# sonbui25/Multimodal-Aspect-Category-Sentiment-Analysis

Hardware: AMD Instinct MI355X
Metric: train samples/sec (fwd+bwd+step) FCMF seq128x36ROI (higher is better)
Workload: dtype bf16; 1 GPU; FCMF-base fine-tune step, BASELINE configs[1]: batch 64 reviews x 6 aspects per GPU, seq 128, 7 images x (49 patches + 36 ROIs), precomputed ResNet-152 features, dropout 0.1, clip 1.0 + 4-group AdamW + linear schedule; global_batch=64, per_gpu_batch=64, seq_len=128, parallelism=dp1, sample_unit=1 review = 6 aspect forwards

## Files before the change

multimodal-aspect-category-sentiment-analysis_amd/csrc/attn_mfma.hip:

```cpp
#include "common.h"
#include <cstdlib>

constexpr int AD = 64;
constexpr int AT = 128;
constexpr int TILE_B = AT * AD * 2;

__device__ __forceinline__ int vkey(int r) { return ((r >> 1) & 1) | (((r >> 3) & 1) << 1); }
__device__ __forceinline__ int off64(int r, int c8) { return r * 128 + ((((c8 >> 1) ^ vkey(r))) << 5) + ((c8 & 1) << 4); }
__device__ __forceinline__ int key16(int r) { return ((r & 7) << 1) ^ (((r >> 3) & 1) * 9); }
__device__ __forceinline__ int off128(int r, int ch) { return r * 256 + ((ch ^ key16(r)) << 4); }
__device__ __forceinline__ int offp(int r, int ch) { return r * 256 + ((ch ^ (r & 15)) << 4); }

__device__ __forceinline__ int off64p(int r, int c8) { return r * 128 + ((((c8 >> 1) ^ ((r >> 1) & 3))) << 5) + ((c8 & 1) << 4); }

typedef bf16x4 __attribute__((address_space(3))) * lds_v4_t;

__device__ __forceinline__ void stage_tile(char* lds, const bf16_t* __restrict__ src, int64_t ld, int rows, int tid) {
#pragma unroll
  for (int i = 0; i < 4; ++i) {
    const int c = tid + 256 * i, r = c >> 3, c8 = c & 7;
    uint4 v = make_uint4(0, 0, 0, 0);
    if (r < rows) v = *reinterpret_cast<const uint4*>(src + (int64_t)r * ld + c8 * 8);
    *reinterpret_cast<uint4*>(lds + off64(r, c8)) = v;
  }
}
__device__ __forceinline__ void stage_tile_p(char* lds, const bf16_t* __restrict__ src, int64_t ld, int rows, int tid) {
#pragma unroll
  for (int i = 0; i < 4; ++i) {
    const int c = tid + 256 * i, r = c >> 3, c8 = c & 7;
    uint4 v = make_uint4(0, 0, 0, 0);
    if (r < rows) v = *reinterpret_cast<const uint4*>(src + (int64_t)r * ld + c8 * 8);
    *reinterpret_cast<uint4*>(lds + off64p(r, c8)) = v;
  }
}
__device__ __forceinline__ bf16x8 frag_tr64p(const char* lds, int c0, int s, int lane) {
  const int g4 = lane >> 4, i16 = lane & 15, q4 = i16 >> 2, p = i16 & 3;
  const int r = 32 * s + 4 * g4 + q4, c8 = (c0 >> 3) + (p >> 1);
  bf16x4 lo = __builtin_amdgcn_ds_read_tr16_b64_v4bf16((lds_v4_t)(lds + off64p(r, c8) + (p & 1) * 8));
  bf16x4 hi = __builtin_amdgcn_ds_read_tr16_b64_v4bf16((lds_v4_t)(lds + off64p(r + 16, c8) + (p & 1) * 8));
  bf16x8 o;
  o[0] = lo[0]; o[1] = lo[1]; o[2] = lo[2]; o[3] = lo[3]; o[4] = hi[0]; o[5] = hi[1]; o[6] = hi[2]; o[7] = hi[3];
  return o;
}
struct TileRegs { uint4 v[4]; };
__device__ __forceinline__ TileRegs load_tile(const bf16_t* __restrict__ src, int64_t ld, int rows, int tid) {
  TileRegs t;
#pragma unroll
  for (int i = 0; i < 4; ++i) {
    const int c = tid + 256 * i, r = c >> 3, c8 = c & 7;
    t.v[i] = make_uint4(0, 0, 0, 0);
    if (r < rows) t.v[i] = *reinterpret_cast<const uint4*>(src + (int64_t)r * ld + c8 * 8);
  }
  return t;
}
template <bool PERMUTED>
__device__ __forceinline__ void store_tile(char* lds, const TileRegs& t, int tid) {
#pragma unroll
  for (int i = 0; i < 4; ++i) {
    const int c = tid + 256 * i, r = c >> 3, c8 = c & 7;
    *reinterpret_cast<uint4*>(lds + (PERMUTED ? off64p(r, c8) : off64(r, c8))) = t.v[i];
  }
}
__device__ __forceinline__ bf16x8 frag_row64(const char* lds, int x0, int s, int lane) {
  return *reinterpret_cast<const bf16x8*>(lds + off64(x0 + (lane & 15), 4 * s + (lane >> 4)));
}
__device__ __forceinline__ bf16x8 frag_tr64(const char* lds, int c0, int s, int lane) {
  const int g4 = lane >> 4, i16 = lane & 15, q4 = i16 >> 2, p = i16 & 3;
  const int r = 32 * s + 8 * g4 + q4, c8 = (c0 >> 3) + (p >> 1);
  bf16x4 lo = __builtin_amdgcn_ds_read_tr16_b64_v4bf16((lds_v4_t)(lds + off64(r, c8) + (p & 1) * 8));
  bf16x4 hi = __builtin_amdgcn_ds_read_tr16_b64_v4bf16((lds_v4_t)(lds + off64(r + 4, c8) + (p & 1) * 8));
  bf16x8 o;
  o[0] = lo[0]; o[1] = lo[1]; o[2] = lo[2]; o[3] = lo[3]; o[4] = hi[0]; o[5] = hi[1]; o[6] = hi[2]; o[7] = hi[3];
  return o;
}
__device__ __forceinline__ bf16x8 frag_row128(const char* lds, int x0, int s, int lane) {
  return *reinterpret_cast<const bf16x8*>(lds + off128(x0 + (lane & 15), 4 * s + (lane >> 4)));
}
__device__ __forceinline__ bf16x8 frag_tr128(const char* lds, int c0, int s, int lane) {
  const int g4 = lane >> 4, i16 = lane & 15, q4 = i16 >> 2, p = i16 & 3;
  const int r = 32 * s + 8 * g4 + q4, ch = (c0 >> 3) + (p >> 1);
  bf16x4 lo = __builtin_amdgcn_ds_read_tr16_b64_v4bf16((lds_v4_t)(lds + off128(r, ch) + (p & 1) * 8));
  bf16x4 hi = __builtin_amdgcn_ds_read_tr16_b64_v4bf16((lds_v4_t)(lds + off128(r + 4, ch) + (p & 1) * 8));
  bf16x8 o;
  o[0] = lo[0]; o[1] = lo[1]; o[2] = lo[2]; o[3] = lo[3]; o[4] = hi[0]; o[5] = hi[1]; o[6] = hi[2]; o[7] = hi[3];
  return o;
}
__device__ __forceinline__ void store4(bf16_t* p, f32x4 v) {
  bf16x4 o;
  o[0] = (bf16_t)v[0]; o[1] = (bf16_t)v[1]; o[2] = (bf16_t)v[2]; o[3] = (bf16_t)v[3];
  *reinterpret_cast<bf16x4*>(p) = o;
}

__device__ __forceinline__ float row16_sum(float x) {
#define FCMF_ROR_ADD(n) x += __builtin_bit_cast(float, __builtin_amdgcn_update_dpp(0, __builtin_bit_cast(int, x), 0x120 + (n), 0xf, 0xf, true))
  FCMF_ROR_ADD(8); FCMF_ROR_ADD(4); FCMF_ROR_ADD(2); FCMF_ROR_ADD(1);
#undef FCMF_ROR_ADD
  return x;
}

struct AttnMfmaParams {
  const bf16_t *q, *k, *v, *o, *dout;
  const float* mask;
  bf16_t *out, *dq, *dk, *dv;
  float* lse;
  float* colsum;
  int G, heads, Tq, Tk;
  int64_t ldq, ldk, ldo;
  float scale, p;
  uint64_t seed;
};

__device__ __forceinline__ void load_q_frags(const AttnMfmaParams& P, int g, int h, int q0, int lane, bf16x8 (&qf)[2][2]) {
#pragma unroll
  for (int f = 0; f < 2; ++f)
#pragma unroll
    for (int s = 0; s < 2; ++s) {
      const int row = q0 + 16 * f + (lane & 15);
      uint4 v = make_uint4(0, 0, 0, 0);
      if (row < P.Tq) v = *reinterpret_cast<const uint4*>(P.q + ((int64_t)g * P.Tq + row) * P.ldq + h * AD + 32 * s + 8 * (lane >> 4));
      qf[f][s] = *reinterpret_cast<bf16x8*>(&v);
    }
}

template <int NKT>
__device__ __forceinline__ void attn_mfma_fwd_tile(const AttnMfmaParams& P, int g, int h, int q0, int lane, const bf16x8 (&qf)[2][2],
                                                   const char* Ks, const char* Vs, const float* mask_lds = nullptr) {
  constexpr int NKF = 8 * NKT;
  const float* mrow = P.mask ? P.mask + (int64_t)g * P.Tk : nullptr;
  int nvalid = P.Tk;
  if (mask_lds || mrow) {
    int last = -1;
#pragma unroll
    for (int i = 0; i < 2 * NKT; ++i) {
      const int key = 64 * i + lane;
      const bool live = key < P.Tk && (mask_lds ? mask_lds[key] : mrow[key]) > -1e30f;
      const unsigned long long b = __ballot(live);
      if (b) last = 64 * i + 63 - __builtin_clzll(b);
    }
    nvalid = last >= 0 ? last + 1 : P.Tk;
  }
  f32x4 sc[NKF][2];
#pragma unroll
  for (int kf = 0; kf < NKF; ++kf)
#pragma unroll
    for (int f = 0; f < 2; ++f) sc[kf][f] = f32x4{0.f, 0.f, 0.f, 0.f};
#pragma unroll
  for (int s = 0; s < 2; ++s)
#pragma unroll
    for (int kf = 0; kf < NKF; ++kf) {
      if (16 * kf >= nvalid) continue;
      const bf16x8 ka = frag_row64(Ks, 16 * kf, s, lane);
#pragma unroll
      for (int f = 0; f < 2; ++f) sc[kf][f] = __builtin_amdgcn_mfma_f32_16x16x32_bf16(ka, qf[f][s], sc[kf][f], 0, 0, 0);
    }
  const float inv_keep = P.p > 0.f ? 1.0f / (1.0f - P.p) : 1.0f;
#pragma unroll
  for (int f = 0; f < 2; ++f) {
    const int q = q0 + 16 * f + (lane & 15);
    float m = -INFINITY;
#pragma unroll
    for (int kf = 0; kf < NKF; ++kf) {
// ... 275 lines not shown
  for (int c = 0; c < nchunks; ++c) {
    f32x4 aV[2], aK[2];
#pragma unroll
    for (int kf = 0; kf < 2; ++kf) { aV[kf] = f32x4{0.f, 0.f, 0.f, 0.f}; aK[kf] = f32x4{0.f, 0.f, 0.f, 0.f}; }
#pragma unroll
    for (int qt = 0; qt < NQT; ++qt) {
      f32x4 sS[2][2], sP[2][2];
#pragma unroll
      for (int k4 = 0; k4 < 2; ++k4)
#pragma unroll
        for (int f = 0; f < 2; ++f) { sS[k4][f] = f32x4{0.f, 0.f, 0.f, 0.f}; sP[k4][f] = f32x4{0.f, 0.f, 0.f, 0.f}; }
#pragma unroll
      for (int s = 0; s < 2; ++s)
#pragma unroll
        for (int k4 = 0; k4 < 2; ++k4) {
          const bf16x8 kb = frag_row64(Ks, 32 * c + 16 * k4, s, lane);
          const bf16x8 vb = frag_row64(Vs, 32 * c + 16 * k4, s, lane);
#pragma unroll
          for (int f = 0; f < 2; ++f) {
            sS[k4][f] = __builtin_amdgcn_mfma_f32_16x16x32_bf16(qa[qt][f][s], kb, sS[k4][f], 0, 0, 0);
            sP[k4][f] = __builtin_amdgcn_mfma_f32_16x16x32_bf16(da[qt][f][s], vb, sP[k4][f], 0, 0, 0);
          }
        }
#pragma unroll
      for (int k4 = 0; k4 < 2; ++k4) {
        const int kl = 16 * k4 + (lane & 15), key = 32 * c + kl;
        const float mk = (mrow && key < P.Tk) ? mrow[key] : 0.f;
#pragma unroll
        for (int f = 0; f < 2; ++f) {
          f32x4 pdv, dsv;
          float mult4[4] = {1.0f, 1.0f, 1.0f, 1.0f};
          if (share_hash) {
            const unsigned q0 = qt * AT + 32 * w + 16 * f + 4 * (lane >> 4);
            const uint32_t o0 = pb_lo + __umul24(q0 + 2 * odd, (unsigned)P.Tk >> 1) + ((unsigned)key >> 1);
            const uint32_t hA = fcmf_hash32_rounds(o0 ^ hash_k0, hash_s1);
            const uint32_t hB = fcmf_hash32_rounds((o0 + ((unsigned)P.Tk >> 1)) ^ hash_k0, hash_s1);
            const uint32_t nA = (uint32_t)__builtin_amdgcn_update_dpp(0, (int)hA, 0xB1, 0xf, 0xf, true);
            const uint32_t nB = (uint32_t)__builtin_amdgcn_update_dpp(0, (int)hB, 0xB1, 0xf, 0xf, true);
            const uint32_t hr[4] = {odd ? nA : hA, odd ? nB : hB, odd ? hA : nA, odd ? hB : nB};
#pragma unroll
            for (int r = 0; r < 4; ++r) mult4[r] = ((hr[r] >> (16 * odd)) & 0xFFFFu) >= drop_thr ? inv_keep : 0.f;
          }
#pragma unroll
          for (int r = 0; r < 4; ++r) {
            const int q = qt * AT + 32 * w + 16 * f + 4 * (lane >> 4) + r;
            float pr = 0.f, mult = mult4[r];
            if (key < P.Tk && q < P.Tq) pr = __expf(sS[k4][f][r] * score_scale + mk - lse4[qt][f][r]);
            if (P.p > 0.f && !share_hash) mult = dropout_mult(P.seed, drop_base + (__umul24((unsigned)q, (unsigned)P.Tk) + (unsigned)key), P.p, inv_keep);
            pdv[r] = pr * mult;
            dsv[r] = pr * (sP[k4][f][r] * mult - dl4[qt][f][r]);
          }
          const int ch = 4 * w + 2 * f + (lane >> 5);
          const int o = off128(kl, ch) + ((lane >> 4) & 1) * 8;
          store4(reinterpret_cast<bf16_t*>(PdT + o), pdv);
          store4(reinterpret_cast<bf16_t*>(dST + o), dsv);
        }
      }
      __syncthreads();
      {
        bf16x8 tb[2];
#pragma unroll
        for (int f = 0; f < 2; ++f) tb[f] = frag_tr128(dST, 32 * w + 16 * f, 0, lane);
#pragma unroll
        for (int df = 0; df < 4; ++df) {
          const bf16x8 ka2 = frag_tr64(Ks, 16 * df, c, lane);
#pragma unroll
          for (int f = 0; f < 2; ++f) aQ[qt][df][f] = __builtin_amdgcn_mfma_f32_16x16x32_bf16(ka2, tb[f], aQ[qt][df][f], 0, 0, 0);
        }
      }
#pragma unroll
      for (int s = 0; s < 4; ++s)
#pragma unroll
        for (int kf = 0; kf < 2; ++kf) {
          const bf16x8 pb = frag_row128(PdT, 16 * kf, s, lane);
          const bf16x8 sb = frag_row128(dST, 16 * kf, s, lane);
          aV[kf] = __builtin_amdgcn_mfma_f32_16x16x32_bf16(oT[qt][s], pb, aV[kf], 0, 0, 0);
          aK[kf] = __builtin_amdgcn_mfma_f32_16x16x32_bf16(qT[qt][s], sb, aK[kf], 0, 0, 0);
        }
      __syncthreads();
    }
    const int dcol = h * AD + 16 * w + 4 * (lane >> 4);
    cV += aV[0] + aV[1];
    cK += aK[0] + aK[1];
#pragma unroll
    for (int kf = 0; kf < 2; ++kf) {
      const int key = 32 * c + 16 * kf + (lane & 15);
      if (key < P.Tk) {
        store4(P.dv + (kbase + key) * P.ldk + dcol, aV[kf]);
        f32x4 t = aK[kf];
        t[0] *= P.scale; t[1] *= P.scale; t[2] *= P.scale; t[3] *= P.scale;
        store4(P.dk + (kbase + key) * P.ldk + dcol, t);
      }
    }
  }
  for (int c = nchunks; c < nchunks_all; ++c) {
    const int dcol = h * AD + 16 * w + 4 * (lane >> 4);
#pragma unroll
    for (int kf = 0; kf < 2; ++kf) {
      const int key = 32 * c + 16 * kf + (lane & 15);
      if (key < P.Tk) {
        store4(P.dv + (kbase + key) * P.ldk + dcol, f32x4{0.f, 0.f, 0.f, 0.f});
        store4(P.dk + (kbase + key) * P.ldk + dcol, f32x4{0.f, 0.f, 0.f, 0.f});
      }
    }
  }
#pragma unroll
  for (int qt = 0; qt < NQT; ++qt)
#pragma unroll
    for (int f = 0; f < 2; ++f) {
      const int x = qt * AT + 32 * w + 16 * f + (lane & 15);
      if (x < P.Tq) {
        const int dcol = h * AD + 4 * (lane >> 4);
#pragma unroll
        for (int df = 0; df < 4; ++df) {
          f32x4 t = aQ[qt][df][f];
          t[0] *= P.scale; t[1] *= P.scale; t[2] *= P.scale; t[3] *= P.scale;
          store4(P.dq + (qbase + x) * P.ldq + dcol + 16 * df, t);
        }
      }
    }
  if (P.colsum) {
    const int HD = P.heads * AD;
    float* row = P.colsum + (int64_t)g * 3 * HD + h * AD;
#pragma unroll
    for (int r = 0; r < 4; ++r) { cV[r] = row16_sum(cV[r]); cK[r] = row16_sum(cK[r]); }
    if ((lane & 15) == 0) {
      const int d0 = 16 * w + 4 * (lane >> 4);
#pragma unroll
      for (int r = 0; r < 4; ++r) { row[2 * HD + d0 + r] = cV[r]; row[HD + d0 + r] = cK[r] * P.scale; }
    }
    float* red = reinterpret_cast<float*>(PdT);
#pragma unroll
    for (int df = 0; df < 4; ++df) {
      f32x4 t = f32x4{0.f, 0.f, 0.f, 0.f};
#pragma unroll
      for (int qt = 0; qt < NQT; ++qt)
#pragma unroll
        for (int f = 0; f < 2; ++f) t += aQ[qt][df][f];
#pragma unroll
      for (int r = 0; r < 4; ++r) t[r] = row16_sum(t[r]);
      if ((lane & 15) == 0) {
#pragma unroll
        for (int r = 0; r < 4; ++r) red[w * 64 + 16 * df + 4 * (lane >> 4) + r] = t[r];
      }
    }
    __syncthreads();
    if (tid < 64) row[tid] = (red[tid] + red[64 + tid] + red[128 + tid] + red[192 + tid]) * P.scale;
  }
}

__global__ __launch_bounds__(256, 2) void attn_mfma_bwd_kernel(AttnMfmaParams P) { attn_mfma_bwd_body<1, 1>(P); }
__global__ __launch_bounds__(256, 1) void attn_mfma_bwd256_kernel(AttnMfmaParams P) { attn_mfma_bwd_body<2, 2>(P); }

static bool al16(const void* p) { return (reinterpret_cast<uintptr_t>(p) & 15) == 0; }

extern "C" int fcmf_attn_mfma_fwd(const void* q, const void* k, const void* v, const float* mask, void* out, float* lse,
                                  int G, int heads, int Tq, int Tk, int64_t ldq, int64_t ldk, int64_t ldo, float scale,
                                  float dropout_p, uint64_t seed, void* stream) {
  if (!q || !k || !v || !out || G <= 0 || heads <= 0 || Tq <= 0 || Tk <= 0) return FCMF_ERR_ARG;
  if (Tk > 2 * AT || ldq % 8 || ldk % 8 || ldo % 4 || !al16(q) || !al16(k) || !al16(v) || !al16(out)) return FCMF_ERR_UNSUPPORTED;
  AttnMfmaParams P{};
  P.q = (const bf16_t*)q; P.k = (const bf16_t*)k; P.v = (const bf16_t*)v; P.mask = mask; P.out = (bf16_t*)out; P.lse = lse;
  P.G = G; P.heads = heads; P.Tq = Tq; P.Tk = Tk; P.ldq = ldq; P.ldk = ldk; P.ldo = ldo;
  P.scale = scale; P.p = dropout_p; P.seed = seed;
  const dim3 grid(G * heads, (Tq + AT - 1) / AT);
  if (Tk > AT) {
    const int smem = 4 * TILE_B;
    static bool attr2 = false;
    return fcmf_launch_flagged(&attr2, attn_mfma_fwd256_kernel, grid, dim3(256), smem, reinterpret_cast<hipStream_t>(stream), P);
  }
  const int ntiles = (int)(grid.x * grid.y);
  static const bool no_persist = getenv("FCMF_ATTN_NO_PERSIST") != nullptr;
  if (ntiles >= 4 * 512 && !no_persist) {
    const int smem = 2 * (2 * TILE_B + 512);
    static bool attr3 = false;
    return fcmf_launch_flagged(&attr3, attn_mfma_fwd_persist_kernel, dim3(512), dim3(256), smem, reinterpret_cast<hipStream_t>(stream), P, ntiles, (int)grid.y);
  }
  const int smem = 2 * TILE_B;
  static bool attr = false;
  return fcmf_launch_flagged(&attr, attn_mfma_fwd_kernel, grid, dim3(256), smem, reinterpret_cast<hipStream_t>(stream), P);
}

extern "C" int fcmf_attn_mfma_bwd(const void* q, const void* k, const void* v, const float* mask, const void* out,
                                  const void* dout, const float* lse, void* dq, void* dk, void* dv, int G, int heads,
                                  int Tq, int Tk, int64_t ldq, int64_t ldk, int64_t ldo, float scale, float dropout_p,
                                  uint64_t seed, float* colsum, void* stream) {
  if (!q || !k || !v || !out || !dout || !lse || !dq || !dk || !dv || G <= 0 || heads <= 0 || Tq <= 0 || Tk <= 0) return FCMF_ERR_ARG;
  if (Tk > 2 * AT || Tq > 2 * AT || ldq % 8 || ldk % 8 || ldo % 8 || !al16(q) || !al16(k) || !al16(v) || !al16(out) || !al16(dout) ||
      !al16(dq) || !al16(dk) || !al16(dv))
    return FCMF_ERR_UNSUPPORTED;
  AttnMfmaParams P{};
  P.q = (const bf16_t*)q; P.k = (const bf16_t*)k; P.v = (const bf16_t*)v; P.mask = mask; P.o = (const bf16_t*)out;
  P.dout = (const bf16_t*)dout; P.lse = const_cast<float*>(lse); P.dq = (bf16_t*)dq; P.dk = (bf16_t*)dk; P.dv = (bf16_t*)dv;
  P.G = G; P.heads = heads; P.Tq = Tq; P.Tk = Tk; P.ldq = ldq; P.ldk = ldk; P.ldo = ldo;
  P.scale = scale; P.p = dropout_p; P.seed = seed; P.colsum = colsum;
  if (Tk > AT || Tq > AT) {
    const int smem = 9 * TILE_B;
    static bool attr2 = false;
    return fcmf_launch_flagged(&attr2, attn_mfma_bwd256_kernel, dim3(G * heads), dim3(256), smem, reinterpret_cast<hipStream_t>(stream), P);
  }
  const int smem = 5 * TILE_B;
  static bool attr = false;
  return fcmf_launch_flagged(&attr, attn_mfma_bwd_kernel, dim3(G * heads), dim3(256), smem, reinterpret_cast<hipStream_t>(stream), P);
}
```

multimodal-aspect-category-sentiment-analysis_amd/csrc/common.h:

```cpp
#pragma once
#include <hip/hip_runtime.h>
#include <stdint.h>
#include "../../include/fcmf_hip.h"

typedef __bf16 bf16_t;
typedef __bf16 bf16x8 __attribute__((ext_vector_type(8)));
typedef __bf16 bf16x4 __attribute__((ext_vector_type(4)));
typedef float f32x4 __attribute__((ext_vector_type(4)));
typedef float f32x16 __attribute__((ext_vector_type(16)));

#define FCMF_CHECK_LAUNCH()                                            \
  do {                                                                 \
    hipError_t e__ = hipGetLastError();                                \
    if (e__ != hipSuccess) return FCMF_ERR_LAUNCH;                     \
  } while (0)

template <class... P, class... A>
static int fcmf_launch_flagged(bool* attr_set, void (*k)(P...), dim3 grid, dim3 block, size_t smem, hipStream_t st, A&&... args) {
  if (smem && !(attr_set && *attr_set)) {
    (void)hipFuncSetAttribute(reinterpret_cast<const void*>(k), hipFuncAttributeMaxDynamicSharedMemorySize, (int)smem);
    if (attr_set) *attr_set = true;
  }
  hipLaunchKernelGGL(k, grid, block, smem, st, static_cast<P>(args)...);
  FCMF_CHECK_LAUNCH();
  return FCMF_OK;
}
template <class... P, class... A>
static int fcmf_launch(void (*k)(P...), dim3 grid, dim3 block, size_t smem, hipStream_t st, A&&... args) {
  return fcmf_launch_flagged(nullptr, k, grid, block, smem, st, args...);
}

template <typename T> __device__ __forceinline__ float to_f32(T x);
template <> __device__ __forceinline__ float to_f32<float>(float x) { return x; }
template <> __device__ __forceinline__ float to_f32<bf16_t>(bf16_t x) { return (float)x; }
template <typename T> __device__ __forceinline__ T from_f32(float x);
template <> __device__ __forceinline__ float from_f32<float>(float x) { return x; }
template <> __device__ __forceinline__ bf16_t from_f32<bf16_t>(float x) { return (bf16_t)x; }

template <typename T> struct Vec4;
template <> struct Vec4<float> {
  typedef float4 raw;
  static __device__ __forceinline__ raw load_raw(const float* p) { return *reinterpret_cast<const float4*>(p); }
  static __device__ __forceinline__ float4 cvt(raw v) { return v; }
  static __device__ __forceinline__ float4 load(const float* p) { return *reinterpret_cast<const float4*>(p); }
  static __device__ __forceinline__ void store(float* p, float4 v) { *reinterpret_cast<float4*>(p) = v; }
};
template <> struct Vec4<bf16_t> {
  typedef bf16x4 raw;
  static __device__ __forceinline__ raw load_raw(const bf16_t* p) { return *reinterpret_cast<const bf16x4*>(p); }
  static __device__ __forceinline__ float4 cvt(raw v) { return make_float4((float)v[0], (float)v[1], (float)v[2], (float)v[3]); }
  static __device__ __forceinline__ float4 load(const bf16_t* p) {
    bf16x4 v = *reinterpret_cast<const bf16x4*>(p);
    return make_float4((float)v[0], (float)v[1], (float)v[2], (float)v[3]);
  }
  static __device__ __forceinline__ void store(bf16_t* p, float4 v) {
    bf16x4 o;
    o[0] = (bf16_t)v.x; o[1] = (bf16_t)v.y; o[2] = (bf16_t)v.z; o[3] = (bf16_t)v.w;
    *reinterpret_cast<bf16x4*>(p) = o;
  }
};

__device__ __forceinline__ float wave_sum(float v) {
#pragma unroll
  for (int o = 32; o > 0; o >>= 1) v += __shfl_xor(v, o, 64);
  return v;
}
__device__ __forceinline__ float wave_max(float v) {
#pragma unroll
  for (int o = 32; o > 0; o >>= 1) v = fmaxf(v, __shfl_xor(v, o, 64));
  return v;
}
__device__ __forceinline__ double wave_sum_d(double v) {
#pragma unroll
  for (int o = 32; o > 0; o >>= 1) v += __shfl_xor(v, o, 64);
  return v;
}

__device__ __forceinline__ uint32_t fcmf_hash32_rounds(uint32_t x, uint32_t s1) {
  x ^= x >> 16; x *= 0x7feb352du;
  x ^= s1;
  x ^= x >> 15; x *= 0x846ca68bu;
  x ^= x >> 16;
  return x;
}
__device__ __forceinline__ uint32_t fcmf_hash32(uint64_t seed, uint64_t pair) {
  const uint32_t s0 = (uint32_t)seed, s1 = (uint32_t)(seed >> 32);
  const uint32_t lo = (uint32_t)pair, hi = (uint32_t)(pair >> 32);
  return fcmf_hash32_rounds(lo ^ s0 ^ ((hi << 7) | (hi >> 25)), s1);
}
__device__ __forceinline__ uint32_t dropout_threshold(float p) { return (uint32_t)(p * 65536.0f + 0.5f); }
__device__ __forceinline__ float dropout_mult(uint64_t seed, uint64_t idx, float p, float inv_keep) {
  const uint32_t h = fcmf_hash32(seed, idx >> 1);
  const uint32_t bits = (idx & 1) ? (h >> 16) : (h & 0xFFFFu);
  return bits >= dropout_threshold(p) ? inv_keep : 0.0f;
}
__device__ __forceinline__ void dropout_mult4(uint64_t seed, uint64_t base, float p, float inv_keep, float (&m)[4]) {
  const uint32_t thr = dropout_threshold(p);
  const uint64_t k0 = base >> 1;
  const uint32_t h0 = fcmf_hash32(seed, k0), h1 = fcmf_hash32(seed, k0 + 1);
  if ((base & 1) == 0) {
    m[0] = (h0 & 0xFFFFu) >= thr ? inv_keep : 0.f; m[1] = (h0 >> 16) >= thr ? inv_keep : 0.f;
    m[2] = (h1 & 0xFFFFu) >= thr ? inv_keep : 0.f; m[3] = (h1 >> 16) >= thr ? inv_keep : 0.f;
  } else {
    const uint32_t h2 = fcmf_hash32(seed, k0 + 2);
    m[0] = (h0 >> 16) >= thr ? inv_keep : 0.f;     m[1] = (h1 & 0xFFFFu) >= thr ? inv_keep : 0.f;
    m[2] = (h1 >> 16) >= thr ? inv_keep : 0.f;     m[3] = (h2 & 0xFFFFu) >= thr ? inv_keep : 0.f;
  }
}

__device__ __forceinline__ float gelu_f(float x) { return x * 0.5f * (1.0f + erff(x * 0.70710678118654752440f)); }
__device__ __forceinline__ float dgelu_f(float x) {
  float cdf = 0.5f * (1.0f + erff(x * 0.70710678118654752440f));
  float pdf = 0.39894228040143267794f * __expf(-0.5f * x * x);
  return cdf + x * pdf;
}
```

multimodal-aspect-category-sentiment-analysis_amd/csrc/gemm.hip:

```cpp
#include "common.h"
#include <cstdio>

struct GemmParams {
  const void* A; const void* B; void* C; const float* bias; void* aux;
  int M, N, K;
  int64_t lda, ldb, ldc;
  int epilogue, accumulate, ksplit, ktiles_per_split;
  unsigned a_bytes, b_bytes;
  unsigned c_bytes;
  float* colsum;
  int tiles, total_items;
  float* ws;
  int nt_out;
  const float* sa; const float* sb;
  int cv_C, cv_logC, cv_Hp, cv_Wp, cv_Ho, cv_Wo, cv_kw, cv_inv_kw, cv_stride;
  float* colstats;
  int cv_logP;
  int tiles_per_mat;
};
constexpr int BATCH_MAX = 32;
struct BatchPtrs { const void* A[BATCH_MAX]; const void* B[BATCH_MAX]; void* C[BATCH_MAX]; };

__device__ __forceinline__ int64_t conv_row_base(const GemmParams& p, int row) {
  const int hw = p.cv_Ho * p.cv_Wo, n = row / hw, rem = row - n * hw, oy = rem / p.cv_Wo, ox = rem - oy * p.cv_Wo;
  return (((int64_t)n * p.cv_Hp + oy * p.cv_stride) * p.cv_Wp + ox * p.cv_stride) << p.cv_logP;
}
__device__ __forceinline__ unsigned conv_k_offset(const GemmParams& p, int kk) {
  const int tap = kk >> p.cv_logC, c0 = kk & (p.cv_C - 1);
  const int ky = (tap * p.cv_inv_kw) >> 16, kx = tap - ky * p.cv_kw;
  return (unsigned)((((ky * p.cv_Wp + kx) << p.cv_logP) + c0) * 2);
}

typedef float f32x2 __attribute__((ext_vector_type(2)));
typedef unsigned u32x4 __attribute__((ext_vector_type(4)));
typedef unsigned u32x2 __attribute__((ext_vector_type(2)));
__device__ __forceinline__ f32x2 splat2(float c) { return f32x2{c, c}; }
__device__ __forceinline__ f32x2 clamp2(f32x2 x, float lim) {
  return f32x2{__builtin_amdgcn_fmed3f(x[0], -lim, lim), __builtin_amdgcn_fmed3f(x[1], -lim, lim)};
}
__device__ __forceinline__ f32x4 clamp4(f32x4 x, float lim) {
  return f32x4{__builtin_amdgcn_fmed3f(x[0], -lim, lim), __builtin_amdgcn_fmed3f(x[1], -lim, lim),
               __builtin_amdgcn_fmed3f(x[2], -lim, lim), __builtin_amdgcn_fmed3f(x[3], -lim, lim)};
}
__device__ __forceinline__ f32x4 splat4(float c) { return f32x4{c, c, c, c}; }
__device__ __forceinline__ f32x4 phi_poly4(f32x4 x) {
  const f32x4 xc = clamp4(x, 4.0f), t = xc * xc;
  f32x4 p = splat4(-1.304578543e-09f);
  p = p * t + splat4(1.060087872e-07f); p = p * t + splat4(-3.746289010e-06f); p = p * t + splat4(7.662426288e-05f);
  p = p * t + splat4(-1.023770734e-03f); p = p * t + splat4(9.590060957e-03f); p = p * t + splat4(-6.607606400e-02f);
  p = p * t + splat4(3.988102128e-01f);
  return xc * p + splat4(0.5f);
}
__device__ __forceinline__ f32x4 dgelu_poly4(f32x4 x) {
  const f32x4 xc = clamp4(x, 4.5f), t = xc * xc;
  f32x4 p = splat4(-2.396099311e-11f);
  p = p * t + splat4(2.702686828e-09f); p = p * t + splat4(-1.343048027e-07f); p = p * t + splat4(3.892256086e-06f);
  p = p * t + splat4(-7.353425424e-05f); p = p * t + splat4(9.596712397e-04f); p = p * t + splat4(-8.909952021e-03f);
  p = p * t + splat4(5.886488750e-02f); p = p * t + splat4(-2.652524630e-01f); p = p * t + splat4(7.977590902e-01f);
  return xc * p + splat4(0.5f);
}
__device__ __forceinline__ f32x2 phi_poly2(f32x2 x) { const f32x4 r = phi_poly4(f32x4{x[0], x[1], x[0], x[1]}); return f32x2{r[0], r[1]}; }
__device__ __forceinline__ f32x2 dgelu_poly2(f32x2 x) { const f32x4 r = dgelu_poly4(f32x4{x[0], x[1], x[0], x[1]}); return f32x2{r[0], r[1]}; }
__device__ __forceinline__ float gelu_poly(float x) { const f32x2 v{x, x}; return (v * phi_poly2(v))[0]; }
__device__ __forceinline__ float dgelu_poly(float x) { return dgelu_poly2(f32x2{x, x})[0]; }
__device__ __forceinline__ float apply_epilogue_fast(float v, int epi, float auxv) {
  switch (epi) {
    case FCMF_EPI_GELU: return gelu_poly(v);
    case FCMF_EPI_TANH: return tanhf(v);
    case FCMF_EPI_DGELU: return v * dgelu_poly(auxv);
    case FCMF_EPI_DTANH: return v * (1.0f - auxv * auxv);
    case FCMF_EPI_ADD: return v + auxv;
    default: return v;
  }
}

__device__ __forceinline__ float apply_epilogue(float v, int epi, float auxv) {
  switch (epi) {
    case FCMF_EPI_GELU: return gelu_f(v);
    case FCMF_EPI_TANH: return tanhf(v);
    case FCMF_EPI_DGELU: return v * dgelu_f(auxv);
    case FCMF_EPI_DTANH: return v * (1.0f - auxv * auxv);
    case FCMF_EPI_ADD: return v + auxv;
    default: return v;
  }
}

constexpr int BM = 128, BN = 128, BK = 32;
constexpr int NSTAGE = 4;
constexpr int TILE_BYTES = 128 * BK * 2;
constexpr int STAGE_BYTES = 2 * TILE_BYTES;

typedef __attribute__((address_space(3))) void* lds_void_t;

__device__ __forceinline__ int swz_row(int r) { return ((r >> 3) & 1) << 1; }
__device__ __forceinline__ int tr_key(int kk) { return (kk & 3) | (((kk >> 3) & 1) << 2); }

template <bool TR>
__device__ __forceinline__ unsigned dma_voffset(int wave, int j, int lane, int64_t ld, int x0, int xdim) {
  const int q = (wave * 2 + j) * 64 + lane;
  if (!TR) {
    const int row = q >> 2, c = (q & 3) ^ swz_row(row);
    if (x0 + row >= xdim) return 0x80000000u;
    return (unsigned)(((int64_t)(x0 + row) * ld + c * 8) * 2);
  } else {
    const int kk = q >> 4, cp = q & 15;
    const int c16 = ((((cp >> 1) ^ tr_key(kk))) << 1) | (cp & 1);
    if (x0 + c16 * 8 >= xdim) return 0x80000000u;
    return (unsigned)(((int64_t)kk * ld + x0 + c16 * 8) * 2);
  }
}


__device__ __forceinline__ u32x4 rsrc_words(const void* p, unsigned bytes) {
  const unsigned long long a = reinterpret_cast<unsigned long long>(p);
  return u32x4{(unsigned)a, (unsigned)(a >> 32) & 0xFFFFu, bytes, 0x00020000u};
}
__device__ __forceinline__ unsigned lds_addr_of(const void* p) {
  return (unsigned)reinterpret_cast<unsigned long long>((__attribute__((address_space(3))) const char*)p);
}
__device__ __forceinline__ void dma16_asm(const u32x4& rsrc, unsigned lds_dst, unsigned voffset, unsigned soffset) {
  asm volatile("s_mov_b32 m0, %0\n\ts_nop 0\n\tbuffer_load_dwordx4 %1, %2, %3 offen lds"
               :: "s"(lds_dst), "v"(voffset), "s"(rsrc), "s"(soffset) : "memory");
}
__device__ __forceinline__ void dma16_asm0(const u32x4& rsrc, unsigned lds_dst, unsigned voffset) {
  asm volatile("s_mov_b32 m0, %0\n\ts_nop 0\n\tbuffer_load_dwordx4 %1, %2, 0 offen lds"
               :: "s"(lds_dst), "v"(voffset), "s"(rsrc) : "memory");
}

template <bool TR>
__device__ __forceinline__ bf16x8 read_frag(const char* lds, int x0, int lane) {
  if (!TR) {
    const int r = x0 + (lane & 15);
    return *reinterpret_cast<const bf16x8*>(lds + r * 64 + ((((lane >> 4)) ^ swz_row(r)) << 4));
  } else {
    const int g = lane >> 4, i16 = lane & 15, q = i16 >> 2, p = i16 & 3;
    const int kk = 8 * g + q, f = x0 >> 4;
    const int off = kk * 256 + ((f ^ tr_key(kk)) << 5) + ((p >> 1) << 4) + ((p & 1) << 3);
    typedef bf16x4 __attribute__((address_space(3))) * lds_v4;
    bf16x4 lo = __builtin_amdgcn_ds_read_tr16_b64_v4bf16((lds_v4)(lds + off));
    bf16x4 hi = __builtin_amdgcn_ds_read_tr16_b64_v4bf16((lds_v4)(lds + off + 4 * 256));
    bf16x8 r;
    r[0] = lo[0]; r[1] = lo[1]; r[2] = lo[2]; r[3] = lo[3];
    r[4] = hi[0]; r[5] = hi[1]; r[6] = hi[2]; r[7] = hi[3];
    return r;
  }
}

template <bool A_TR, bool B_TR, typename TC>
__global__ __launch_bounds__(256, 2) void gemm_bf16_kernel(GemmParams p) {
  extern __shared__ __attribute__((aligned(16))) char smem[];
  const int tid = threadIdx.x, lane = tid & 63;
  const int wave = __builtin_amdgcn_readfirstlane(tid >> 6);
  const int wm = wave >> 1, wn = wave & 1;

  const int tiles_n = (p.N + BN - 1) / BN;
  const int nblk = gridDim.x;
  int bid = blockIdx.x;
  {
    int q = nblk >> 3, r = nblk & 7, xcd = bid & 7, local = bid >> 3;
    bid = (xcd < r ? xcd * (q + 1) : r * (q + 1) + (xcd - r) * q) + local;
  }
  const int tile_m = bid / tiles_n, tile_n = bid % tiles_n;
  const int i0 = tile_m * BM, j0 = tile_n * BN;

  const int nk_total = (p.K + BK - 1) / BK;
  const int kt_begin = blockIdx.z * p.ktiles_per_split;
  const int kt_end = min(nk_total, kt_begin + p.ktiles_per_split);
  const int nkt = kt_end - kt_begin;

  const __amdgpu_buffer_rsrc_t rA = __builtin_amdgcn_make_buffer_rsrc(const_cast<void*>(p.A), 0, p.a_bytes, 0x00020000);
  const __amdgpu_buffer_rsrc_t rB = __builtin_amdgcn_make_buffer_rsrc(const_cast<void*>(p.B), 0, p.b_bytes, 0x00020000);
  unsigned va[2], vb[2];
#pragma unroll
  for (int j = 0; j < 2; ++j) {
    va[j] = dma_voffset<A_TR>(wave, j, lane, p.lda, i0, p.M);
    vb[j] = dma_voffset<B_TR>(wave, j, lane, p.ldb, j0, p.N);
    if constexpr (!A_TR) {
      if (p.cv_C) {
        const int q = (wave * 2 + j) * 64 + lane, row = q >> 2, c = (q & 3) ^ swz_row(row);
        va[j] = i0 + row < p.M ? (unsigned)((conv_row_base(p, i0 + row) + c * 8) * 2) : 0x80000000u;
      }
    }
  }
  const unsigned a_step = A_TR ? (unsigned)(BK * p.lda * 2) : (unsigned)(BK * 2);
  const unsigned b_step = B_TR ? (unsigned)(BK * p.ldb * 2) : (unsigned)(BK * 2);

  constexpr bool ASM_DMA = A_TR || B_TR;
  [[maybe_unused]] const u32x4 wA = rsrc_words(p.A, p.a_bytes), wB = rsrc_words(p.B, p.b_bytes);
  auto issue = [&](int t) {
    char* st = smem + (t & (NSTAGE - 1)) * STAGE_BYTES + (wave * 2) * 1024;
    const unsigned ka = (!A_TR && p.cv_C) ? conv_k_offset(p, (kt_begin + t) * BK) : (unsigned)(kt_begin + t) * a_step;
    const unsigned kb = (unsigned)(kt_begin + t) * b_step;
#pragma unroll
    for (int j = 0; j < 2; ++j) {
      if constexpr (ASM_DMA) {
        if (A_TR) dma16_asm0(wA, lds_addr_of(st + j * 1024), va[j] + ka);
        else      dma16_asm(wA, lds_addr_of(st + j * 1024), va[j], ka);
        if (B_TR) dma16_asm0(wB, lds_addr_of(st + TILE_BYTES + j * 1024), vb[j] + kb);
        else      dma16_asm(wB, lds_addr_of(st + TILE_BYTES + j * 1024), vb[j], kb);
      } else {
        __builtin_amdgcn_raw_ptr_buffer_load_lds(rA, (lds_void_t)(st + j * 1024), 16, va[j], ka, 0, 0);
        __builtin_amdgcn_raw_ptr_buffer_load_lds(rB, (lds_void_t)(st + TILE_BYTES + j * 1024), 16, vb[j], kb, 0, 0);
      }
    }
  };

  f32x4 acc[4][4];
#pragma unroll
  for (int a = 0; a < 4; ++a)
#pragma unroll
    for (int b = 0; b < 4; ++b) acc[a][b] = f32x4{0.f, 0.f, 0.f, 0.f};

#pragma unroll
  for (int t = 0; t < NSTAGE - 1; ++t)
    if (t < nkt) issue(t);

  for (int t = 0; t < nkt; ++t) {
    const int younger = nkt - 1 - t;
    if (younger >= 2) asm volatile("s_waitcnt vmcnt(8)" ::: "memory");
    else if (younger == 1) asm volatile("s_waitcnt vmcnt(4)" ::: "memory");
    else asm volatile("s_waitcnt vmcnt(0)" ::: "memory");
    __builtin_amdgcn_s_barrier();
    if (t + NSTAGE - 1 < nkt) issue(t + NSTAGE - 1);
    const char* la = smem + (t & (NSTAGE - 1)) * STAGE_BYTES;
    const char* lb = la + TILE_BYTES;
    bf16x8 fa[4], fb[4];
#pragma unroll
    for (int f = 0; f < 4; ++f) {
      fa[f] = read_frag<A_TR>(la, wm * 64 + f * 16, lane);
      fb[f] = read_frag<B_TR>(lb, wn * 64 + f * 16, lane);
    }
#pragma unroll
    for (int fj = 0; fj < 4; ++fj)
#pragma unroll
      for (int fi = 0; fi < 4; ++fi)
        acc[fj][fi] = __builtin_amdgcn_mfma_f32_16x16x32_bf16(fb[fj], fa[fi], acc[fj][fi], 0, 0, 0);
  }

  TC* C = reinterpret_cast<TC*>(p.C);
  TC* AUX = reinterpret_cast<TC*>(p.aux);
  const bool atomic = (p.ksplit > 1);
  const bool lead = (blockIdx.z == 0);
  float4 cs[4] = {make_float4(0, 0, 0, 0), make_float4(0, 0, 0, 0), make_float4(0, 0, 0, 0), make_float4(0, 0, 0, 0)};
#pragma unroll
  for (int fi = 0; fi < 4; ++fi) {
    const int i = i0 + wm * 64 + fi * 16 + (lane & 15);
    if (i >= p.M) continue;
#pragma unroll
    for (int fj = 0; fj < 4; ++fj) {
      const int j = j0 + wn * 64 + fj * 16 + (lane >> 4) * 4;
      if (j >= p.N) continue;
      float4 v = make_float4(acc[fj][fi][0], acc[fj][fi][1], acc[fj][fi][2], acc[fj][fi][3]);
      if (p.bias && lead) {
        float4 b = *reinterpret_cast<const float4*>(p.bias + j);
        v.x += b.x; v.y += b.y; v.z += b.z; v.w += b.w;
      }
      const int64_t off = (int64_t)i * p.ldc + j;
      if (p.epilogue != FCMF_EPI_NONE) {
        float4 a = make_float4(0, 0, 0, 0);
        if (p.epilogue == FCMF_EPI_GELU) { if (AUX) Vec4<TC>::store(AUX + off, v); }
        else if (p.epilogue != FCMF_EPI_TANH) a = Vec4<TC>::load(AUX + off);
        if constexpr (sizeof(TC) == 2) {
          v.x = apply_epilogue_fast(v.x, p.epilogue, a.x); v.y = apply_epilogue_fast(v.y, p.epilogue, a.y);
          v.z = apply_epilogue_fast(v.z, p.epilogue, a.z); v.w = apply_epilogue_fast(v.w, p.epilogue, a.w);
        } else {
          v.x = apply_epilogue(v.x, p.epilogue, a.x); v.y = apply_epilogue(v.y, p.epilogue, a.y);
          v.z = apply_epilogue(v.z, p.epilogue, a.z); v.w = apply_epilogue(v.w, p.epilogue, a.w);
        }
      }
      if constexpr (sizeof(TC) == 4) {
        float* cf = reinterpret_cast<float*>(C) + off;
        if (atomic) {
          atomicAdd(cf + 0, v.x); atomicAdd(cf + 1, v.y); atomicAdd(cf + 2, v.z); atomicAdd(cf + 3, v.w);
        } else if (p.accumulate) {
          float4 o = *reinterpret_cast<float4*>(cf);
          o.x += v.x; o.y += v.y; o.z += v.z; o.w += v.w;
          *reinterpret_cast<float4*>(cf) = o;
        } else {
          *reinterpret_cast<float4*>(cf) = v;
        }
// ... 1686 lines not shown
```

Before: 1723 samples/s.

## Add persistent attention backward kernel with cross-item async LDS prefetch

Adds a persistent attention-backward kernel that runs a fixed grid of 512 workgroups looping over (batch, head) items. While one item is computed it issues buffer-to-LDS DMA loads for the next item's Q, dO, K and V tiles, and it loads the next item's O, LSE and mask early. The goal is to hide global-memory latency and remove per-workgroup launch and tail costs when there are many small items. The path only runs when there are at least 2048 items. It adds complexity, environment-variable overrides, and possible races because the next item's tiles are written into LDS that is still being read.

After: 1734 samples/s (median of 6 runs). Within noise of the previous version (+0.7%).

```diff
diff --git a/multimodal-aspect-category-sentiment-analysis_amd/csrc/attn_mfma.hip b/multimodal-aspect-category-sentiment-analysis_amd/csrc/attn_mfma.hip
--- a/multimodal-aspect-category-sentiment-analysis_amd/csrc/attn_mfma.hip
+++ b/multimodal-aspect-category-sentiment-analysis_amd/csrc/attn_mfma.hip
@@ -1,12 +1,11 @@
 #include "common.h"
+#include "attn_swizzle.h"
 #include <cstdlib>
 
 constexpr int AD = 64;
 constexpr int AT = 128;
 constexpr int TILE_B = AT * AD * 2;
 
-__device__ __forceinline__ int vkey(int r) { return ((r >> 1) & 1) | (((r >> 3) & 1) << 1); }
-__device__ __forceinline__ int off64(int r, int c8) { return r * 128 + ((((c8 >> 1) ^ vkey(r))) << 5) + ((c8 & 1) << 4); }
 __device__ __forceinline__ int key16(int r) { return ((r & 7) << 1) ^ (((r >> 3) & 1) * 9); }
 __device__ __forceinline__ int off128(int r, int ch) { return r * 256 + ((ch ^ key16(r)) << 4); }
 __device__ __forceinline__ int offp(int r, int ch) { return r * 256 + ((ch ^ (r & 15)) << 4); }
@@ -588,6 +587,323 @@
 __global__ __launch_bounds__(256, 2) void attn_mfma_bwd_kernel(AttnMfmaParams P) { attn_mfma_bwd_body<1, 1>(P); }
 __global__ __launch_bounds__(256, 1) void attn_mfma_bwd256_kernel(AttnMfmaParams P) { attn_mfma_bwd_body<2, 2>(P); }
 
+__global__ __launch_bounds__(256, 2) void attn_mfma_bwd_persist_kernel(AttnMfmaParams P, int nitems) {
+  extern __shared__ __attribute__((aligned(16))) char smem[];
+  char* Qs = smem;
+  char* dOs = Qs + TILE_B;
+  char* Ks = dOs + TILE_B;
+  char* Vs = Ks + TILE_B;
+  char* PdT = Vs + TILE_B;
+  char* dST = PdT + TILE_B / 2;
+  const int tid = threadIdx.x, lane = tid & 63;
+  const int w = __builtin_amdgcn_readfirstlane(tid >> 6);
+  int item = blockIdx.x;
+  if (item >= nitems) return;
+  int g = item / P.heads, h = item - g * P.heads;
+
+  auto fresh_lane = [&]() { int l = lane; asm volatile("" : "+v"(l)); return l; };
+  auto dma_piece = [&](const u32x4& rs, char* tile, int i, int64_t ld, int rows) {
+    const int ln = fresh_lane(), lr = ln >> 3;
+    const unsigned vo = 8 * i + lr < rows ? (unsigned)((lr * ld + dma_col_piece(8 * w + lr, ln & 7) * 8) * 2) : 0x80000000u;
+    dma16_asm(rs, lds_addr_of(tile + i * 1024), vo, (unsigned)(8 * i * ld * 2));
+  };
+  struct ItemSrc { u32x4 q, dout, k, v; };
+  auto src_of = [&](int gg, int hh) {
+    ItemSrc s;
+    const unsigned qb = (unsigned)(((int64_t)(P.Tq - 1) * P.ldq + AD) * 2), ob = (unsigned)(((int64_t)(P.Tq - 1) * P.ldo + AD) * 2);
+    const unsigned kb = (unsigned)(((int64_t)(P.Tk - 1) * P.ldk + AD) * 2);
+    s.q = rsrc_words(P.q + (int64_t)gg * P.Tq * P.ldq + hh * AD, qb);
+    s.dout = rsrc_words(P.dout + (int64_t)gg * P.Tq * P.ldo + hh * AD, ob);
+    s.k = rsrc_words(P.k + (int64_t)gg * P.Tk * P.ldk + hh * AD, kb);
+    s.v = rsrc_words(P.v + (int64_t)gg * P.Tk * P.ldk + hh * AD, kb);
+    return s;
+  };
+  struct Early { uint4 o[4]; float lse[2][4]; float m0, m1; };
+  auto early_load = [&](int gg, int hh, Early& e) {
+    const int lane = fresh_lane();
+    const int q = 32 * w + (lane >> 1), half = lane & 1;
+#pragma unroll
+    for (int i = 0; i < 4; ++i) e.o[i] = make_uint4(0, 0, 0, 0);
+    if (q < P.Tq) {
+      const bf16_t* b = P.o + ((int64_t)gg * P.Tq + q) * P.ldo + hh * AD + 32 * half;
+#pragma unroll
+      for (int i = 0; i < 4; ++i) e.o[i] = *reinterpret_cast<const uint4*>(b + 8 * i);
+    }
+#pragma unroll
+    for (int f = 0; f < 2; ++f)
+#pragma unroll
+      for (int r = 0; r < 4; ++r) {
+        const int q2 = 32 * w + 16 * f + 4 * (lane >> 4) + r;
+        e.lse[f][r] = q2 < P.Tq ? P.lse[((int64_t)gg * P.heads + hh) * P.Tq + q2] : 0.f;
+      }
+    e.m0 = (P.mask && lane < P.Tk) ? P.mask[(int64_t)gg * P.Tk + lane] : 0.f;
+    e.m1 = (P.mask && 64 + lane < P.Tk) ? P.mask[(int64_t)gg * P.Tk + 64 + lane] : 0.f;
+  };
+
+  Early e;
+  {
+    const ItemSrc s = src_of(g, h);
+#pragma unroll
+    for (int j = 0; j < 4; ++j) {
+      dma_piece(s.q, Qs, w + 4 * j, P.ldq, P.Tq);
+      dma_piece(s.dout, dOs, w + 4 * j, P.ldo, P.Tq);
+      dma_piece(s.k, Ks, w + 4 * j, P.ldk, P.Tk);
+      dma_piece(s.v, Vs, w + 4 * j, P.ldk, P.Tk);
+    }
+    early_load(g, h, e);
+  }
+
+  const float inv_keep = P.p > 0.f ? 1.0f / (1.0f - P.p) : 1.0f;
+  const uint32_t drop_thr = dropout_threshold(P.p);
+  const int odd = lane & 1;
+  const int nchunks_all = (P.Tk + 31) >> 5;
+  for (;;) {
+    asm volatile("s_waitcnt vmcnt(0)" ::: "memory");
+    __syncthreads();
+    const int64_t qbase = (int64_t)g * P.Tq, kbase = (int64_t)g * P.Tk;
+    float dl4[2][4], lse4[2][4];
+    {
+      const int q = 32 * w + (lane >> 1), half = lane & 1;
+      float sd = 0.f;
+      if (q < P.Tq) {
+#pragma unroll
+        for (int i = 0; i < 4; ++i) {
+          const bf16x8 x = *reinterpret_cast<const bf16x8*>(dOs + off64(q, 4 * half + i));
+          const bf16x8 y = *reinterpret_cast<const bf16x8*>(&e.o[i]);
+#pragma unroll
+          for (int j = 0; j < 8; ++j) sd += (float)x[j] * (float)y[j];
+        }
+      }
+      sd += __shfl_xor(sd, 1, 64);
+#pragma unroll
+      for (int f = 0; f < 2; ++f)
+#pragma unroll
+        for (int r = 0; r < 4; ++r) {
+          dl4[f][r] = __shfl(sd, 2 * (16 * f + 4 * (lane >> 4) + r), 64);
+          lse4[f][r] = e.lse[f][r];
+        }
+    }
+    float m0 = e.m0, m1 = e.m1;
+    bf16x8 qa[2][2], da[2][2], oT[4], qT[4];
+    f32x4 aQ[4][2];
+#pragma unroll
+    for (int f = 0; f < 2; ++f)
+#pragma unroll
+      for (int s = 0; s < 2; ++s) {
+        qa[f][s] = frag_row64(Qs, 32 * w + 16 * f, s, lane);
+        da[f][s] = frag_row64(dOs, 32 * w + 16 * f, s, lane);
+      }
+#pragma unroll
+    for (int s = 0; s < 4; ++s) {
+      oT[s] = frag_tr64(dOs, 16 * w, s, lane);
+      qT[s] = frag_tr64(Qs, 16 * w, s, lane);
+    }
+#pragma unroll
+    for (int df = 0; df < 4; ++df)
+#pragma unroll
+      for (int f = 0; f < 2; ++f) aQ[df][f] = f32x4{0.f, 0.f, 0.f, 0.f};
+
+    const int nxt = item + gridDim.x;
+    const bool more = nxt < nitems;
+    const int g2 = more ? nxt / P.heads : g, h2 = more ? nxt - g2 * P.heads : h;
+    const ItemSrc sn = src_of(g2, h2);
+
+    const uint64_t drop_base = ((uint64_t)g * P.heads + h) * P.Tq * P.Tk;
+    float score_scale = P.scale;
+    int nvalid = P.Tk;
+    if (P.mask) {
+      int last = -1;
+#pragma unroll
+      for (int i = 0; i < 2; ++i) {
+        const int key = 64 * i + lane;
+        const bool live = key < P.Tk && (i ? m1 : m0) > -1e30f;
+        const unsigned long long b = __ballot(live);
+        if (b) last = 64 * i + 63 - __builtin_clzll(b);
+      }
+      nvalid = last >= 0 ? last + 1 : P.Tk;
+      if (last < 0) {
+        m0 = 0.f; m1 = 0.f;
+        score_scale = 0.f;
+        const float ltk = __logf((float)P.Tk);
+#pragma unroll
+        for (int f = 0; f < 2; ++f)
+#pragma unroll
+          for (int r = 0; r < 4; ++r) lse4[f][r] = ltk;
+      }
+    }
+    const int nchunks = (nvalid + 31) >> 5;
+    const uint64_t pair_base = drop_base >> 1;
+    const uint32_t pb_lo = (uint32_t)pair_base, pb_hi = (uint32_t)(pair_base >> 32);
+    const bool share_hash = P.p > 0.f && (P.Tk & 1) == 0 && pb_lo <= 0xFFFF0000u;
+    const uint32_t hash_k0 = (uint32_t)P.seed ^ ((pb_hi << 7) | (pb_hi >> 25)), hash_s1 = (uint32_t)(P.seed >> 32);
+    f32x4 cV = f32x4{0.f, 0.f, 0.f, 0.f}, cK = f32x4{0.f, 0.f, 0.f, 0.f};
+    const int dcol = h * AD + 16 * w + 4 * (fresh_lane() >> 4);
+    for (int c = 0; c < nchunks; ++c) {
+      f32x4 aV[2], aK[2];
+#pragma unroll
+      for (int kf = 0; kf < 2; ++kf) { aV[kf] = f32x4{0.f, 0.f, 0.f, 0.f}; aK[kf] = f32x4{0.f, 0.f, 0.f, 0.f}; }
+      f32x4 sS[2][2], sP[2][2];
+#pragma unroll
+      for (int k4 = 0; k4 < 2; ++k4)
+#pragma unroll
+        for (int f = 0; f < 2; ++f) { sS[k4][f] = f32x4{0.f, 0.f, 0.f, 0.f}; sP[k4][f] = f32x4{0.f, 0.f, 0.f, 0.f}; }
+#pragma unroll
+      for (int s = 0; s < 2; ++s)
+#pragma unroll
+        for (int k4 = 0; k4 < 2; ++k4) {
+          const bf16x8 kb = frag_row64(Ks, 32 * c + 16 * k4, s, lane);
+          const bf16x8 vb = frag_row64(Vs, 32 * c + 16 * k4, s, lane);
+#pragma unroll
+          for (int f = 0; f < 2; ++f) {
+            sS[k4][f] = __builtin_amdgcn_mfma_f32_16x16x32_bf16(qa[f][s], kb, sS[k4][f], 0, 0, 0);
+            sP[k4][f] = __builtin_amdgcn_mfma_f32_16x16x32_bf16(da[f][s], vb, sP[k4][f], 0, 0, 0);
+          }
+        }
+      const float mhalf = c >= 2 ? m1 : m0;
+#pragma unroll
+      for (int k4 = 0; k4 < 2; ++k4) {
+        const int kl = 16 * k4 + (lane & 15), key = 32 * c + kl;
+        const float mk = __shfl(mhalf, key & 63, 64);
+#pragma unroll
+        for (int f = 0; f < 2; ++f) {
+          f32x4 pdv, dsv;
+          float mult4[4] = {1.0f, 1.0f, 1.0f, 1.0f};
+          if (share_hash) {
+            const unsigned q0 = 32 * w + 16 * f + 4 * (lane >> 4);
+            const uint32_t o0 = pb_lo + __umul24(q0 + 2 * odd, (unsigned)P.Tk >> 1) + ((unsigned)key >> 1);
+            const uint32_t hA = fcmf_hash32_rounds(o0 ^ hash_k0, hash_s1);
+            const uint32_t hB = fcmf_hash32_rounds((o0 + ((unsigned)P.Tk >> 1)) ^ hash_k0, hash_s1);
+            const uint32_t nA = (uint32_t)__builtin_amdgcn_update_dpp(0, (int)hA, 0xB1, 0xf, 0xf, true);
+            const uint32_t nB = (uint32_t)__builtin_amdgcn_update_dpp(0, (int)hB, 0xB1, 0xf, 0xf, true);
+            const uint32_t hr[4] = {odd ? nA : hA, odd ? nB : hB, odd ? hA : nA, odd ? hB : nB};
+#pragma unroll
+            for (int r = 0; r < 4; ++r) mult4[r] = ((hr[r] >> (16 * odd)) & 0xFFFFu) >= drop_thr ? inv_keep : 0.f;
+          }
+#pragma unroll
+          for (int r = 0; r < 4; ++r) {
+            const int q = 32 * w + 16 * f + 4 * (lane >> 4) + r;
+            float pr = 0.f, mult = mult4[r];
+            if (key < P.Tk && q < P.Tq) pr = __expf(sS[k4][f][r] * score_scale + mk - lse4[f][r]);
+            if (P.p > 0.f && !share_hash) mult = dropout_mult(P.seed, drop_base + (__umul24((unsigned)q, (unsigned)P.Tk) + (unsigned)key), P.p, inv_keep);
+            pdv[r] = pr * mult;
+            dsv[r] = pr * (sP[k4][f][r] * mult - dl4[f][r]);
+          }
+          const int ch = 4 * w + 2 * f + (lane >> 5);
+          const int o = off128(kl, ch) + ((lane >> 4) & 1) * 8;
+          store4(reinterpret_cast<bf16_t*>(PdT + o), pdv);
+          store4(reinterpret_cast<bf16_t*>(dST + o), dsv);
+        }
+      }
+      __syncthreads();
+      {
+        bf16x8 tb[2];
+#pragma unroll
+        for (int f = 0; f < 2; ++f) tb[f] = frag_tr128(dST, 32 * w + 16 * f, 0, lane);
+#pragma unroll
+        for (int df = 0; df < 4; ++df) {
+          const bf16x8 ka2 = frag_tr64(Ks, 16 * df, c, lane);
+#pragma unroll
+          for (int f = 0; f < 2; ++f) aQ[df][f] = __builtin_amdgcn_mfma_f32_16x16x32_bf16(ka2, tb[f], aQ[df][f], 0, 0, 0);
+        }
+      }
+#pragma unroll
+      for (int s = 0; s < 4; ++s)
+#pragma unroll
+        for (int kf = 0; kf < 2; ++kf) {
+          const bf16x8 pb = frag_row128(PdT, 16 * kf, s, lane);
+          const bf16x8 sb = frag_row128(dST, 16 * kf, s, lane);
+          aV[kf] = __builtin_amdgcn_mfma_f32_16x16x32_bf16(oT[s], pb, aV[kf], 0, 0, 0);
+          aK[kf] = __builtin_amdgcn_mfma_f32_16x16x32_bf16(qT[s], sb, aK[kf], 0, 0, 0);
+        }
+      __syncthreads();
+      if (more) {
+        dma_piece(sn.k, Ks, 4 * c + w, P.ldk, P.Tk);
+        dma_piece(sn.v, Vs, 4 * c + w, P.ldk, P.Tk);
+        if (c == 0) {
+#pragma unroll
+          for (int j = 0; j < 4; ++j) {
+            dma_piece(sn.q, Qs, w + 4 * j, P.ldq, P.Tq);
+            dma_piece(sn.dout, dOs, w + 4 * j, P.ldo, P.Tq);
+          }
+          for (int cc = nchunks; cc < 4; ++cc) {
+            dma_piece(sn.k, Ks, 4 * cc + w, P.ldk, P.Tk);
+            dma_piece(sn.v, Vs, 4 * cc + w, P.ldk, P.Tk);
+          }
+        }
+      }
+      cV += aV[0] + aV[1];
+      cK += aK[0] + aK[1];
+#pragma unroll
+      for (int kf = 0; kf < 2; ++kf) {
+        const int key = 32 * c + 16 * kf + (lane & 15);
+        if (key < P.Tk) {
+          store4(P.dv + (kbase + key) * P.ldk + dcol, aV[kf]);
+          f32x4 t = aK[kf];
+          t[0] *= P.scale; t[1] *= P.scale; t[2] *= P.scale; t[3] *= P.scale;
+          store4(P.dk + (kbase + key) * P.ldk + dcol, t);
+        }
+      }
+    }
+    for (int c = nchunks; c < nchunks_all; ++c) {
+      const int lane = fresh_lane();
+      const int dcol = h * AD + 16 * w + 4 * (lane >> 4);
+#pragma unroll
+      for (int kf = 0; kf < 2; ++kf) {
+        const int key = 32 * c + 16 * kf + (lane & 15);
+        if (key < P.Tk) {
+          store4(P.dv + (kbase + key) * P.ldk + dcol, f32x4{0.f, 0.f, 0.f, 0.f});
+          store4(P.dk + (kbase + key) * P.ldk + dcol, f32x4{0.f, 0.f, 0.f, 0.f});
+        }
+      }
+    }
+    early_load(g2, h2, e);
+    {
+    const int lane = fresh_lane();
+#pragma unroll
+    for (int f = 0; f < 2; ++f) {
+      const int x = 32 * w + 16 * f + (lane & 15);
+      if (x < P.Tq) {
+        const int dcol = h * AD + 4 * (lane >> 4);
+#pragma unroll
+        for (int df = 0; df < 4; ++df) {
+          f32x4 t = aQ[df][f];
+          t[0] *= P.scale; t[1] *= P.scale; t[2] *= P.scale; t[3] *= P.scale;
+          store4(P.dq + (qbase + x) * P.ldq + dcol + 16 * df, t);
+        }
+      }
+    }
+    if (P.colsum) {
+      const int HD = P.heads * AD;
+      float* row = P.colsum + (int64_t)g * 3 * HD + h * AD;
+#pragma unroll
+      for (int r = 0; r < 4; ++r) { cV[r] = row16_sum(cV[r]); cK[r] = row16_sum(cK[r]); }
+      if ((lane & 15) == 0) {
+        const int d0 = 16 * w + 4 * (lane >> 4);
+#pragma unroll
+        for (int r = 0; r < 4; ++r) { row[2 * HD + d0 + r] = cV[r]; row[HD + d0 + r] = cK[r] * P.scale; }
+      }
+      float* red = reinterpret_cast<float*>(PdT);
+#pragma unroll
+      for (int df = 0; df < 4; ++df) {
+        f32x4 t = f32x4{0.f, 0.f, 0.f, 0.f};
+#pragma unroll
+        for (int f = 0; f < 2; ++f) t += aQ[df][f];
+#pragma unroll
+        for (int r = 0; r < 4; ++r) t[r] = row16_sum(t[r]);
+        if ((lane & 15) == 0) {
+#pragma unroll
+          for (int r = 0; r < 4; ++r) red[w * 64 + 16 * df + 4 * (lane >> 4) + r] = t[r];
+        }
+      }
+      __syncthreads();
+      if (w == 0) row[lane] = (red[lane] + red[64 + lane] + red[128 + lane] + red[192 + lane]) * P.scale;
+    }
+    }
+    if (!more) break;
+    item = nxt; g = g2; h = h2;
+  }
+}
+
 static bool al16(const void* p) { return (reinterpret_cast<uintptr_t>(p) & 15) == 0; }
 
 extern "C" int fcmf_attn_mfma_fwd(const void* q, const void* k, const void* v, const float* mask, void* out, float* lse,
@@ -636,6 +952,15 @@
     return fcmf_launch_flagged(&attr2, attn_mfma_bwd256_kernel, dim3(G * heads), dim3(256), smem, reinterpret_cast<hipStream_t>(stream), P);
   }
   const int smem = 5 * TILE_B;
+  const int nitems = G * heads;
+  const char* grid_env = getenv("FCMF_ATTN_BWD_PERSIST_GRID");
+  const int grid_forced = grid_env ? atoi(grid_env) : 0;
+  const bool fits = ldq <= (1 << 22) && ldk <= (1 << 22) && ldo <= (1 << 22);
+  if (fits && !getenv("FCMF_ATTN_BWD_NO_PERSIST") && (grid_forced > 0 || nitems >= 4 * 512)) {
+    const int nwg = grid_forced > 0 ? (grid_forced < nitems ? grid_forced : nitems) : 512;
+    static bool attr3 = false;
+    return fcmf_launch_flagged(&attr3, attn_mfma_bwd_persist_kernel, dim3(nwg), dim3(256), smem, reinterpret_cast<hipStream_t>(stream), P, nitems);
+  }
   static bool attr = false;
   return fcmf_launch_flagged(&attr, attn_mfma_bwd_kernel, dim3(G * heads), dim3(256), smem, reinterpret_cast<hipStream_t>(stream), P);
 }
diff --git a/multimodal-aspect-category-sentiment-analysis_amd/csrc/attn_swizzle.h b/multimodal-aspect-category-sentiment-analysis_amd/csrc/attn_swizzle.h
--- /dev/null
+++ b/multimodal-aspect-category-sentiment-analysis_amd/csrc/attn_swizzle.h
@@ -0,0 +1,13 @@
+#pragma once
+#if defined(__HIPCC__) || defined(__CUDACC__)
+#define FCMF_HD __host__ __device__ __forceinline__
+#else
+#define FCMF_HD inline
+#endif
+
+FCMF_HD int vkey(int r) { return ((r >> 1) & 1) | (((r >> 3) & 1) << 1); }
+FCMF_HD int off64(int r, int c8) { return r * 128 + ((((c8 >> 1) ^ vkey(r))) << 5) + ((c8 & 1) << 4); }
+
+FCMF_HD int dma_row(int i, int lane) { return 8 * i + (lane >> 3); }
+FCMF_HD int dma_col_piece(int r, int pc) { return (((pc >> 1) ^ vkey(r)) << 1) | (pc & 1); }
+FCMF_HD int dma_lds_byte(int i, int lane) { return (64 * i + lane) * 16; }
diff --git a/multimodal-aspect-category-sentiment-analysis_amd/csrc/common.h b/multimodal-aspect-category-sentiment-analysis_amd/csrc/common.h
--- a/multimodal-aspect-category-sentiment-analysis_amd/csrc/common.h
+++ b/multimodal-aspect-category-sentiment-analysis_amd/csrc/common.h
@@ -28,6 +28,24 @@
 template <class... P, class... A>
 static int fcmf_launch(void (*k)(P...), dim3 grid, dim3 block, size_t smem, hipStream_t st, A&&... args) {
   return fcmf_launch_flagged(nullptr, k, grid, block, smem, st, args...);
+}
+
+typedef unsigned u32x4 __attribute__((ext_vector_type(4)));
+
+__device__ __forceinline__ u32x4 rsrc_words(const void* p, unsigned bytes) {
+  const unsigned long long a = reinterpret_cast<unsigned long long>(p);
+  return u32x4{(unsigned)a, (unsigned)(a >> 32) & 0xFFFFu, bytes, 0x00020000u};
+}
+__device__ __forceinline__ unsigned lds_addr_of(const void* p) {
+  return (unsigned)reinterpret_cast<unsigned long long>((__attribute__((address_space(3))) const char*)p);
+}
+__device__ __forceinline__ void dma16_asm(const u32x4& rsrc, unsigned lds_dst, unsigned voffset, unsigned soffset) {
+  asm volatile("s_mov_b32 m0, %0\n\ts_nop 0\n\tbuffer_load_dwordx4 %1, %2, %3 offen lds"
+               :: "s"(lds_dst), "v"(voffset), "s"(rsrc), "s"(soffset) : "memory");
+}
+__device__ __forceinline__ void dma16_asm0(const u32x4& rsrc, unsigned lds_dst, unsigned voffset) {
+  asm volatile("s_mov_b32 m0, %0\n\ts_nop 0\n\tbuffer_load_dwordx4 %1, %2, 0 offen lds"
+               :: "s"(lds_dst), "v"(voffset), "s"(rsrc) : "memory");
 }
 
 template <typename T> __device__ __forceinline__ float to_f32(T x);
diff --git a/multimodal-aspect-category-sentiment-analysis_amd/csrc/gemm.hip b/multimodal-aspect-category-sentiment-analysis_amd/csrc/gemm.hip
--- a/multimodal-aspect-category-sentiment-analysis_amd/csrc/gemm.hip
+++ b/multimodal-aspect-category-sentiment-analysis_amd/csrc/gemm.hip
@@ -32,7 +32,6 @@
 }
 
 typedef float f32x2 __attribute__((ext_vector_type(2)));
-typedef unsigned u32x4 __attribute__((ext_vector_type(4)));
 typedef unsigned u32x2 __attribute__((ext_vector_type(2)));
 __device__ __forceinline__ f32x2 splat2(float c) { return f32x2{c, c}; }
 __device__ __forceinline__ f32x2 clamp2(f32x2 x, float lim) {
@@ -111,21 +110,6 @@
 }
 
 
-__device__ __forceinline__ u32x4 rsrc_words(const void* p, unsigned bytes) {
-  const unsigned long long a = reinterpret_cast<unsigned long long>(p);
-  return u32x4{(unsigned)a, (unsigned)(a >> 32) & 0xFFFFu, bytes, 0x00020000u};
-}
-__device__ __forceinline__ unsigned lds_addr_of(const void* p) {
-  return (unsigned)reinterpret_cast<unsigned long long>((__attribute__((address_space(3))) const char*)p);
-}
-__device__ __forceinline__ void dma16_asm(const u32x4& rsrc, unsigned lds_dst, unsigned voffset, unsigned soffset) {
-  asm volatile("s_mov_b32 m0, %0\n\ts_nop 0\n\tbuffer_load_dwordx4 %1, %2, %3 offen lds"
-               :: "s"(lds_dst), "v"(voffset), "s"(rsrc), "s"(soffset) : "memory");
-}
-__device__ __forceinline__ void dma16_asm0(const u32x4& rsrc, unsigned lds_dst, unsigned voffset) {
-  asm volatile("s_mov_b32 m0, %0\n\ts_nop 0\n\tbuffer_load_dwordx4 %1, %2, 0 offen lds"
-               :: "s"(lds_dst), "v"(voffset), "s"(rsrc) : "memory");
-}
 
 template <bool TR>
 __device__ __forceinline__ bf16x8 read_frag(const char* lds, int x0, int lane) {
```
